# claussss/ubisoft-laforge-daft-exprt

Measured on AMD Instinct MI355X. Metric: mel frames/sec (fwd+bwd), higher is better.
Workload: dtype bf16; 1 GPU; C2: LJ-shaped training step, 48 utterances/GPU, L_max=120, T_max=896, 28180 valid frames/GPU/step; forward + loss (mel L1/L2, adversarial CE, post-mult, energy + pitch consistency) + backward + fused Adam step (global-norm clip, LR schedule) + one-launch weight re-pack, dropout on; parallelism=dp1, launch=1 captured HIP graph(s) per step (one per backward phase) + eager optimiser

## Files before the change

### include/daft_exprt_hip.h

```cpp
#ifndef DAFT_EXPRT_HIP_H
#define DAFT_EXPRT_HIP_H

#include <stdint.h>

#ifdef __cplusplus
extern "C" {
#endif

int dx_version(void);
const char* dx_last_error(void);
int dx_prof_enable(int kind, int capacity);
int dx_prof_collect(int kind, int* launches, double* total_ms);

int dx_int_durations(const float* dur, int B, int L, int sampling_rate, int filter_length, int hop_length, int centered,
                     long long* out, long long* totals, int* status);

int dx_pack_dims(int Cout, int Cin, int bf16, int* dims);
int dx_pack_weights(const float* W, void* fwd, void* bwd, int Cout, int Cin, int taps, int bf16, void* stream);
int dx_pack_weights_batched(const void* descs, int n, int bf16, void* stream);
int dx_pack_weights_host(const void* descs, int n, int bf16, void* stream);
int dx_conv_gemm(const void* X, int ldx, const void* Wp, const float* bias, void* Y, int ldy,
                 int B, int N, int Cin, int Cout, int taps, int bf16,
                 int relu, const float* post_scale, const float* post_shift,
                 const void* relu_aux, int ld_aux, int accumulate,
// ... 26 lines not shown
                     uint64_t seed_pre, float p_pre, const uint64_t* seed_offset, void* stream);
int dx_ff_block_bwd(const float* dY2, const float* z2, const float* mean2, const float* rstd2, const float* ln2_w, const float* ln2_b,
                    const float* film, int ld_film, void* DG2, float* dw2, float* db2, float* dfilm, int ld_dfilm, uint64_t seed2, float p2,
                    const void* Wa, const void* Wb, const void* aux, int ld_aux, void* H, int ldh, float* Y,
                    int B, int N, int F, const int* lens, int skip_halo,
                    const float* z1, const float* mean1, const float* rstd1, const float* ln1_w, const float* ln1_b, void* DG1, float* dw1, float* db1,
                    uint64_t seed1, float p1, const void* Wout_bwd, void* DATT, const uint64_t* seed_offset, const void* hmask,
                    const int* rows_exist, void* stream);
int dx_colsum(const void* X, int ldx, float* out, long rows, int C, int x_bf16, void* stream);

int dx_length_order(const int* lens, int* order, int B, void* stream);
int dx_attention_fwd(const void* qkv, int ld, const int* lens, void* ctx, int ldc, float* lse,
                     int B, int N, int H, int D, uint64_t seed, const uint64_t* seed_offset, float p_drop, int bf16, int qkv_bf16, int ctx_bf16,
                     const int* order, void* stream);
int dx_attention_proj_ln_fwd(const void* qkv, int ld, const int* lens, void* ctx, int ldc, float* lse, int B, int N, int H, int D,
                             uint64_t seed, const uint64_t* seed_offset, float p_drop,
                             const void* Wpack, const float* proj_bias, float* z, const float* res, const float* w, const float* bias,
                             const float* film, int ld_film, float* y, float* mean, float* rstd, uint64_t seed_pre, float p_pre,
                             void* y_bf16_copy, void* stream);
int dx_attention_bwd(const void* qkv, int ld, const void* ctx, const void* dctx, int ldc, const float* lse, float* delta,
                     const int* lens, void* dqkv, int ldg, int B, int N, int H, int D, uint64_t seed, const uint64_t* seed_offset, float p_drop, int bf16,
                     int qkv_bf16, int dqkv_bf16, int ctx_bf16, const int* order, void* stream);

int dx_ln_fwd(void* a, const void* res, const float* w, const float* bias, const float* film, int ld_film,
              const int* lens, int halo, void* y, float* mean, float* rstd, int B, int N, int C,
              uint64_t seed_pre, float p_pre, uint64_t seed_post, float p_post, const uint64_t* seed_offset, int io_bf16, void* y_bf16_copy,
              void* stream);
int dx_film_affine_fwd(const float* gammas, const float* betas, const float* pm, float* film, int B, int nb, int C, void* stream);
int dx_film_affine_bwd(const void* dfilm_ptrs, const float* gammas, const float* betas, const float* pm, float* dgammas, float* dbetas, float* dpm,
                       int B, int nb, int C, void* stream);
int dx_proj_ln_fwd(const void* X, int ldx, const void* Wpack, const float* proj_bias, float* z, const float* res, const float* w, const float* bias,
                   const float* film, int ld_film, const int* lens, int halo, float* y, float* mean, float* rstd, int B, int N,
                   uint64_t seed_pre, float p_pre, const uint64_t* seed_offset, void* y_bf16_copy, void* stream);
int dx_ln_bwd(const void* dy, const void* z, const float* mean, const float* rstd, const float* w, const float* bias,
              const float* film, int ld_film, const int* lens, int halo, void* dz, void* da, float* dw, float* dbias,
              float* dfilm, int ld_dfilm, int B, int N, int C, int relu_mask,
              uint64_t seed_pre, float p_pre, uint64_t seed_post, float p_post, const uint64_t* seed_offset, int io_bf16, void* dg_bf16_copy,
              void* stream);

int dx_add_pos(const float* x, const long* sym, const float* emb, const float* pe, const int* lens, float* out,
               int B, int N, int D, int pe_rows, void* stream);
int dx_mask_rows(const float* in, const int* lens, float* out, int B, int N, int C, void* stream);
int dx_embedding_bwd(const float* dout, const long* sym, const int* lens, float* demb, int B, int N, int D, void* stream);
int dx_accent_sum(const float* prenet, const float* energy, const float* pitch, const float* we, const float* be,
                  const float* wp, const float* bp, const float* pe, const int* lens, float* out,
                  int B, int N, int D, int pe_rows, void* stream);
int dx_scalar_conv_wgrad(const float* dout, int ldd, const float* rowscale, const float* s0, const float* s1, const int* lens,
                         float* dw0, float* db0, float* dw1, float* db1, int B, int N, int D, void* stream);
int dx_mean_pool(const float* x, const int* lens, float* out, int B, int N, int C, void* stream);
int dx_mean_pool_bwd(const float* dout, const int* lens, float* dx, int B, int N, int C, void* stream);
int dx_transpose(const float* in, float* out, int B, int R, int Cc, int accumulate, void* stream);
int dx_relu_bwd(const float* dy, const float* y, float* out, long n, void* stream);
int dx_channel_affine(const void* x, const float* scale, const float* shift, void* out, long rows, int C, int io_bf16, void* stream);
int dx_l2_normalize(const float* x, float* y, int rows, int C, void* stream);
int dx_cross_entropy(const float* logits, const long* target, float* loss, float* dlogits, int B, int S, void* stream);

int dx_duration_scan(const long* dur_int, float* mu, long* totals, int B, int L, void* stream);
int dx_upsample_prep(const float* enc, const float* dur, const float* energy, const float* pitch,
                     const float* wd, const float* bd, const float* we, const float* be, const float* wp, const float* bp,
                     const float* wr, const float* br, const int* lens, float* xs, float* z, float* sigma,
                     int B, int L, int D, void* stream);
int dx_upsample_fwd(const float* xs, const float* mu, const float* sigma, const int* lens, float* weights, float* xup,
                    int B, int L, int T, int D, void* stream);
int dx_upsample_bwd(const float* dxup, const float* xs, const float* mu, const float* sigma, const float* weights, const int* lens,
                    float* dxs, float* dsigma, int B, int L, int T, int D, void* stream);
int dx_upsample_sym_bwd(const float* dxs_in, const float* dsigma, const float* xs, const float* z, const float* dur, const int* lens,
// ... 62 lines not shown
```

### ubisoft_laforge_daft_exprt_amd/csrc/dx_f16_names.h

```cpp
#pragma once
#define dx_accent_sum dx_accent_sum_f16
#define dx_add_pos dx_add_pos_f16
#define dx_attention_bwd dx_attention_bwd_f16
#define dx_attention_fwd dx_attention_fwd_f16
#define dx_attention_proj_ln_fwd dx_attention_proj_ln_fwd_f16
#define dx_channel_affine dx_channel_affine_f16
#define dx_colsum dx_colsum_f16
#define dx_condition_prosody dx_condition_prosody_f16
#define dx_conv_gemm dx_conv_gemm_f16
#define dx_conv_wgrad dx_conv_wgrad_f16
#define dx_conv_wgrad_batched dx_conv_wgrad_batched_f16
#define dx_cross_entropy dx_cross_entropy_f16
#define dx_embedding_bwd dx_embedding_bwd_f16
#define dx_ff_block_bwd dx_ff_block_bwd_f16
#define dx_ff_pair dx_ff_pair_f16
#define dx_ff_pair_ln dx_ff_pair_ln_f16
#define dx_ff_pair_ln_qkv dx_ff_pair_ln_qkv_f16
#define dx_ff_pair_lnbwd dx_ff_pair_lnbwd_f16
#define dx_gather_speaker_rows dx_gather_speaker_rows_f16
#define dx_l2_normalize dx_l2_normalize_f16
#define dx_length_order dx_length_order_f16
#define dx_ln_bwd dx_ln_bwd_f16
#define dx_film_affine_bwd dx_film_affine_bwd_f16
#define dx_film_affine_fwd dx_film_affine_fwd_f16
#define dx_ln_fwd dx_ln_fwd_f16
#define dx_proj_ln_fwd dx_proj_ln_fwd_f16
#define dx_mask_rows dx_mask_rows_f16
#define dx_mean_pool dx_mean_pool_f16
#define dx_mean_pool_bwd dx_mean_pool_bwd_f16
#define dx_pack_dims dx_pack_dims_f16
#define dx_pitch_chain_bwd dx_pitch_chain_bwd_f16
#define dx_pitch_chain_fwd dx_pitch_chain_fwd_f16
#define dx_pack_weights dx_pack_weights_f16
#define dx_pack_weights_batched dx_pack_weights_batched_f16
#define dx_pack_weights_host dx_pack_weights_host_f16
#define dx_relu_bwd dx_relu_bwd_f16
#define dx_scalar_conv_wgrad dx_scalar_conv_wgrad_f16
#define dx_transpose dx_transpose_f16
#define dx_unpack_wgrad dx_unpack_wgrad_f16
```

### ubisoft_laforge_daft_exprt_amd/csrc/dx_gemm.hip

```cpp
#include "dx_common.h"
#include <algorithm>
#include <stdlib.h>
#include <type_traits>

namespace {

constexpr int TILE = 128;
constexpr int DK_MAX_B = 1024;

struct ConvGemmArgs {
  const float* X; int ldx;
  const void* Wp;
  const float* bias;
  float* Y; int ldy;
  int B, N, Cin, Cout, CinP, CoutP;
  int relu;
  const float* post_scale; const float* post_shift;
  const float* relu_aux; int ld_aux;
  int accumulate;
  const int* lens; int mask_rows;
  float out_scale;
  int skip_halo;
  int x_bf16, y_bf16, aux_bf16;
  const int* rows_exist;
// ... 1857 lines not shown
  long rr = r0;
  for (; rr + 3 < r1; rr += 4) {
    s0 += (float)X[(size_t)rr * ldx + c];
    s1 += (float)X[(size_t)(rr + 1) * ldx + c];
    s2 += (float)X[(size_t)(rr + 2) * ldx + c];
    s3 += (float)X[(size_t)(rr + 3) * ldx + c];
  }
  for (; rr < r1; ++rr) s0 += (float)X[(size_t)rr * ldx + c];
  const float t = (s0 + s1) + (s2 + s3);
  if (t != 0.f) atomicAdd(&out[c], t);
}

template <typename T, int TAPS, int TOK, bool XH>
void launch_conv_inst(const ConvGemmArgs& a, hipStream_t s) {
  const size_t smem = (size_t)(TAPS * TILE + TOK + TAPS - 1) * 128;
  static bool configured = false;
  if (!configured) {
    hipFuncSetAttribute(reinterpret_cast<const void*>(&conv_gemm_kernel<T, TAPS, TOK, XH>), hipFuncAttributeMaxDynamicSharedMemorySize, (int)smem);
    configured = true;
  }
  dim3 grid(a.B * dx_cdiv(a.N, TOK), a.CoutP / TILE);
  hipLaunchKernelGGL((conv_gemm_kernel<T, TAPS, TOK, XH>), grid, dim3(256), smem, s, a);
}

template <typename T, int TAPS>
int launch_conv(const ConvGemmArgs& a, hipStream_t s) {
  constexpr long small_below = (sizeof(T) == 4 || TAPS == 1) ? 1024 : 0;
  const bool small = (long)a.B * dx_cdiv(a.N, TILE) * (a.CoutP / TILE) < small_below;
  if constexpr (sizeof(T) == 2) {
    if (a.x_bf16) { if (small) launch_conv_inst<T, TAPS, 64, true>(a, s); else launch_conv_inst<T, TAPS, 128, true>(a, s); return DX_OK; }
  }
  if (small) launch_conv_inst<T, TAPS, 64, false>(a, s); else launch_conv_inst<T, TAPS, 128, false>(a, s);
  return DX_OK;
}

}

extern "C" {

int dx_pack_dims(int Cout, int Cin, int bf16, int* dims) {
  const int bk = bf16 ? 64 : 32;
  dims[0] = dx_roundup(Cout, TILE);
  dims[1] = dx_roundup(Cin, bk);
  dims[2] = dx_roundup(Cin, TILE);
  dims[3] = dx_roundup(Cout, bk);
  return DX_OK;
}

int dx_pack_weights(const float* W, void* fwd, void* bwd, int Cout, int Cin, int taps, int bf16, void* stream) {
  DX_REQUIRE(W && fwd, "dx_pack_weights: null pointer");
  DX_REQUIRE(Cout > 0 && Cin > 0 && (taps == 1 || taps == 3), "dx_pack_weights: bad dims Cout=%d Cin=%d taps=%d", Cout, Cin, taps);
  int d[4];
  dx_pack_dims(Cout, Cin, bf16, d);
  const size_t n = (size_t)taps * d[0] * d[1] + (bwd ? (size_t)taps * d[2] * d[3] : 0);
  const int blocks = (int)std::min<size_t>((n + 255) / 256, 4096);
  hipStream_t s = (hipStream_t)stream;
  if (bf16)
    hipLaunchKernelGGL(pack_weights_kernel<dx_h16>, dim3(blocks), dim3(256), 0, s, W, (dx_h16*)fwd, (dx_h16*)bwd, Cout, Cin, taps, d[0], d[1], d[2], d[3]);
  else
    hipLaunchKernelGGL(pack_weights_kernel<float>, dim3(blocks), dim3(256), 0, s, W, (float*)fwd, (float*)bwd, Cout, Cin, taps, d[0], d[1], d[2], d[3]);
  DX_LAUNCH_CHECK("dx_pack_weights");
  return DX_OK;
}

int dx_pack_weights_batched(const void* descs, int n, int bf16, void* stream) {
  DX_REQUIRE(descs && n > 0, "dx_pack_weights_batched: bad arguments");
// ... 47 lines not shown
  DX_REQUIRE(!aux_bf16 || ((Cout % 4) == 0 && (ld_aux % 4) == 0), "dx_conv_gemm: bf16 relu_aux needs Cout, ld_aux multiples of 4");
  DX_REQUIRE(skip_halo < 0 || lens, "dx_conv_gemm: skip_halo needs lens");
  DX_REQUIRE(B > 0 && N > 0 && Cin > 0 && Cout > 0, "dx_conv_gemm: bad dims B=%d N=%d Cin=%d Cout=%d", B, N, Cin, Cout);
  DX_REQUIRE(taps == 1 || taps == 3, "dx_conv_gemm: taps must be 1 or 3 (got %d)", taps);
  DX_REQUIRE((Cin % 4) == 0 && (ldx % 4) == 0 && ldx >= Cin, "dx_conv_gemm: Cin (%d) and ldx (%d) must be multiples of 4, ldx >= Cin", Cin, ldx);
  DX_REQUIRE(ldy >= Cout && ((Cout % 4) != 0 || (ldy % 4) == 0), "dx_conv_gemm: bad ldy %d for Cout %d", ldy, Cout);
  DX_REQUIRE(((uintptr_t)X % 16) == 0 && ((uintptr_t)Wp % 16) == 0 && ((uintptr_t)Y % 16) == 0, "dx_conv_gemm: pointers must be 16-byte aligned");
  DX_REQUIRE(!relu_aux || ld_aux >= Cout, "dx_conv_gemm: bad ld_aux");
  DX_REQUIRE((post_scale == nullptr) == (post_shift == nullptr), "dx_conv_gemm: post_scale/post_shift must come together");
  DX_REQUIRE(!mask_rows || lens, "dx_conv_gemm: mask_rows needs lens");
  int d[4];
  dx_pack_dims(Cout, Cin, bf16 == 1, d);
  ConvGemmArgs a{X, ldx, Wp, bias, Y, ldy, B, N, Cin, Cout, d[1], d[0], relu, post_scale, post_shift,
                 relu_aux, ld_aux, accumulate, lens, mask_rows, out_scale, skip_halo, x_bf16, y_bf16, aux_bf16, rows_exist};
  hipStream_t s = (hipStream_t)stream;
  dx_prof_begin(DX_PROF_CONV_GEMM, s);
  constexpr int ws_min_tiles = 64;
  constexpr int dk_min_cin = 256;
  if (bf16 == 2) {
    if constexpr (kSplitBuild) { if (taps == 3) launch_conv<dx_split3, 3>(a, s); else launch_conv<dx_split3, 1>(a, s); }
  } else if (bf16 && d[1] >= dk_min_cin && (Cin % 64) == 0 && (long)B * N * ldx < (1L << 31)) {
    if (x_bf16) { if (taps == 3) launch_conv_dk<3, true>(a, s); else launch_conv_dk<1, true>(a, s); }
    else { if (taps == 3) launch_conv_dk<3, false>(a, s); else launch_conv_dk<1, false>(a, s); }
  } else if (bf16 && d[1] == 128 && (long)B * dx_cdiv(N, 128) >= ws_min_tiles) {
    if (x_bf16) { if (taps == 3) launch_conv_ws<3, true>(a, s); else launch_conv_ws<1, true>(a, s); }
    else { if (taps == 3) launch_conv_ws<3, false>(a, s); else launch_conv_ws<1, false>(a, s); }
  } else if (bf16) { if (taps == 3) launch_conv<dx_h16, 3>(a, s); else launch_conv<dx_h16, 1>(a, s); }
  else      { if (taps == 3) launch_conv<float, 3>(a, s);  else launch_conv<float, 1>(a, s); }
  dx_prof_end(DX_PROF_CONV_GEMM, s);
  DX_LAUNCH_CHECK("dx_conv_gemm");
  return DX_OK;
}

int dx_conv_wgrad(const void* dY, int ldy, const void* X, int ldx, float* G,
                  int B, int N, int Cin, int Cout, int taps, const int* lens, int skip_halo,
                  int bf16, int dy_bf16, int x_bf16, float* dbias, const int* rows_exist, void* stream) {
  DX_REQUIRE(dY && X && G, "dx_conv_wgrad: null pointer");
  DX_REQUIRE(bf16 == 0 || bf16 == 1 || (bf16 == 2 && kSplitBuild), "dx_conv_wgrad: bad operand mode %d", bf16);
  DX_REQUIRE(bf16 == 1 || !(dy_bf16 || x_bf16), "dx_conv_wgrad: bf16 storage needs bf16 operand mode");
  const bool bf16_ok = (Cin % 8) == 0 && (ldx % 8) == 0 && (Cout % 8) == 0 && (ldy % 8) == 0;
  DX_REQUIRE(bf16_ok || !(dy_bf16 || x_bf16), "dx_conv_wgrad: bf16-stored operands need Cin/Cout/ld multiples of 8 (Cin=%d Cout=%d)", Cin, Cout);
  if (bf16 == 1 && bf16_ok) {
    DX_REQUIRE(B > 0 && N > 0 && Cin > 0 && Cout > 0 && (taps == 1 || taps == 3), "dx_conv_wgrad: bad dims");
    DX_REQUIRE(((uintptr_t)X % 16) == 0 && ((uintptr_t)dY % 16) == 0, "dx_conv_wgrad: pointers must be 16-byte aligned");
    DX_REQUIRE(skip_halo < 0 || lens, "dx_conv_wgrad: skip_halo needs lens");
    const bool wide = (Cin % 128) == 0 && dx_cdiv(Cout, TILE) * dx_cdiv(Cin, 64) >= 64;
    const int tiles = dx_cdiv(Cout, TILE) * dx_cdiv(Cin, wide ? 128 : 64);
    const int total_chunks = B * dx_cdiv(N, wb_bk(taps, dy_bf16 != 0, x_bf16 != 0));
    constexpr int target_blocks = 256;
    constexpr int target_wide = 256;
    constexpr int target_k1 = 192;
    const int ksplit = std::max(1, std::min(total_chunks, dx_cdiv(wide ? target_wide : (taps == 1 ? target_k1 : target_blocks), tiles)));
    WgradBatchArgs a{};
    a.job[0] = WgradJobDev{dY, X, G, dbias, lens, ldy, ldx, B, N, Cin, Cout, skip_halo, 0, rows_exist};
    a.ksplit = ksplit;
    hipStream_t s = (hipStream_t)stream;
    dim3 grid(tiles, 1, ksplit);
    dx_prof_begin(DX_PROF_WGRAD_GEMM, s);
#define DX_WG_LAUNCH(TAPS_, CIW_)                                                                                        \
    if (dy_bf16 && x_bf16) hipLaunchKernelGGL((wgrad_bf16_kernel<TAPS_, true, true, CIW_>), grid, dim3(CIW_ * 128), 0, s, a);   \
    else if (dy_bf16) hipLaunchKernelGGL((wgrad_bf16_kernel<TAPS_, true, false, CIW_>), grid, dim3(CIW_ * 128), 0, s, a);       \
    else if (x_bf16) hipLaunchKernelGGL((wgrad_bf16_kernel<TAPS_, false, true, CIW_>), grid, dim3(CIW_ * 128), 0, s, a);        \
    else hipLaunchKernelGGL((wgrad_bf16_kernel<TAPS_, false, false, CIW_>), grid, dim3(CIW_ * 128), 0, s, a);
    if (wide) { if (taps == 3) { DX_WG_LAUNCH(3, 4) } else { DX_WG_LAUNCH(1, 4) } }
    else { if (taps == 3) { DX_WG_LAUNCH(3, 2) } else { DX_WG_LAUNCH(1, 2) } }
#undef DX_WG_LAUNCH
// ... 94 lines not shown
```

### ubisoft_laforge_daft_exprt_amd/functional.py

```python
from __future__ import annotations

import threading

import torch

from . import ops

_seed_state = threading.local()


def manual_seed(seed: int) -> None:
    _seed_state.base = (int(seed) * 0x9E3779B97F4A7C15 + 0x1234567) & 0xFFFFFFFFFFFFFFFF
    _seed_state.counter = 0


def next_seed() -> int:
    if not hasattr(_seed_state, 'base'):
        manual_seed(torch.initial_seed())
    _seed_state.counter += 1
    return (_seed_state.base + _seed_state.counter * 0xD1B54A32D192ED03) & 0xFFFFFFFFFFFFFFFF


def _sink(param, enabled):
    if not enabled or param is None:
# ... 197 lines not shown
            dz1, da1, dln1_w, dln1_b = r1[:4]
            dproj = r1[5] if sh else (da1 if da1 is not None else dz1)
        dc1_w, dc1_b = ops.conv_wgrad(dh, y1, packs['c1'], L, 1, arena=arena, w_sink=g('c1_w'), b_sink=g('c1_b'), prec=prec, defer=True, rows_exist=E)
        dout_w, dout_b = ops.conv_wgrad(dproj, att, packs['out'], L, 0, arena=arena, w_sink=g('out_w'), b_sink=g('out_b'), prec=prec, defer=True)
        if datt is None:
            datt = ops.conv_gemm(dproj, packs['out'], None, transpose=True, lens=L, halo=0, prec=prec, out_dtype=att.dtype)
        dqkv = ops.attention_bwd(qkv, att, datt, lse, L, ctx.heads, s_attn, p_attn, out_dtype=qkv.dtype, prec=prec, seed_offset=so)
        din_w, din_b = ops.conv_wgrad(dqkv, x, packs['in'], L, 0, arena=arena, w_sink=g('in_w'), b_sink=g('in_b'), prec=prec, defer=True)
        dx = ops.conv_gemm(dqkv, packs['in'], None, transpose=True, out=dz1, accumulate=True, lens=L, halo=0, prec=prec)
        return (dx, dfilm, None, None, None, None,
                din_w, din_b, dout_w, dout_b, dln1_w, dln1_b, dc1_w, dc1_b, dc2_w, dc2_b, dln2_w, dln2_b, None, None)


def cut(rt, level, t):
    sp = None if rt is None else rt.backward_split
    if sp is None or level > rt.cut_levels or not t.requires_grad:
        return t
    leaf = t.detach().requires_grad_(True)
    sp.append((level, t, leaf))
    return leaf


class AccentFront0Fn(torch.autograd.Function):
    @staticmethod
    def forward(ctx, mel, lens, packs, p_drop, training, c0_w, c0_b, l0_w, l0_b):
        p = p_drop if training else 0.0
        seed = next_seed() if training else 0
        x0 = ops.transpose(mel.contiguous())
        L = lens.i32
        rt = packs['p0'].rt
        prec = rt.precision
        hd = ops.hidden_dtype(prec)
        so = rt.seed_offset
        h0 = ops.conv_gemm(x0, packs['p0'], c0_b, relu=True, lens=L, halo=2, out_dtype=hd, prec=prec, rows_exist=lens.exist)
        y0, m0, r0 = ops.ln_fwd(h0, None, l0_w, l0_b, None, L, seed_post=seed, p_post=p, halo=2, seed_offset=so, prec=prec)
        ctx.save_for_backward(x0, h0, m0, r0, l0_w, l0_b)
        ctx.lens, ctx.packs, ctx.p, ctx.seed = lens, packs, p, seed
        ctx.prec, ctx.sink, ctx.seed_offset = prec, rt.sink, so
        return y0

    @staticmethod
    def backward(ctx, dy0):
        x0, h0, m0, r0, l0_w, l0_b = ctx.saved_tensors
        lens, packs, p = ctx.lens, ctx.packs, ctx.p
        arena = packs['p0'].rt.arena
        L = lens.i32
        sk = {k: _sink(v, ctx.sink) for k, v in packs.get('params', {}).items()}
        g = sk.get
        dz0, _, dl0_w, dl0_b, _ = ops.ln_bwd(dy0.contiguous(), h0, m0, r0, l0_w, l0_b, None, L, relu_mask=True, seed_post=ctx.seed, p_post=p,
                                              seed_offset=ctx.seed_offset, prec=ctx.prec, w_sink=g('l0_w'), b_sink=g('l0_b'), halo=2, arena=arena)
        dc0_w, dc0_b = ops.conv_wgrad(dz0, x0, packs['p0'], L, 2, w_sink=g('c0_w'), b_sink=g('c0_b'), prec=ctx.prec, arena=arena, rows_exist=lens.exist)
        return None, None, None, None, None, dc0_w, dc0_b, dl0_w, dl0_b


class AccentFront12Fn(torch.autograd.Function):
    @staticmethod
    def forward(ctx, y0, energy, pitch, lens, packs, pe, p_drop, training,
                c1_w, c1_b, l1_w, l1_b, c2_w, c2_b, l2_w, l2_b, we, be, wp, bp):
        p = p_drop if training else 0.0
        seeds = [next_seed() if training else 0 for _ in range(2)]
        L = lens.i32
        rt = packs['p1'].rt
        prec = rt.precision
        hd = ops.hidden_dtype(prec)
        so = rt.seed_offset
        h1 = ops.conv_gemm(y0, packs['p1'], c1_b, relu=True, lens=L, halo=1, out_dtype=hd, prec=prec, rows_exist=lens.exist)
        y1, m1, r1 = ops.ln_fwd(h1, None, l1_w, l1_b, None, L, seed_post=seeds[0], p_post=p, halo=1, seed_offset=so, prec=prec)
        h2 = ops.conv_gemm(y1, packs['p2'], c2_b, relu=True, lens=L, halo=0, prec=prec, rows_exist=lens.exist)
# ... 164 lines not shown
```

### ubisoft_laforge_daft_exprt_amd/ops.py

```python
from __future__ import annotations

import ctypes

import torch

from . import _lib
from ._lib import lib

PRECISIONS = ('f32', 'bf16', 'fp16', 'bf16x3')


class Runtime:

    def __init__(self, precision='f32'):
        self.precision = _check_precision(precision)
        self.pack_epoch = 0
        self.sink = False
        self.launch_log = None
        self.arena = None
        self.arena_hint = 1 << 20
        self.seed_offset = None
        self.defer_wgrad = False
        self.wgrad_queue = {}
        self.backward_split = None
# ... 464 lines not shown
    return ctx, lse


def attention_bwd(qkv, ctx, dctx, lse, lens, heads, seed, p_drop, out_dtype=torch.float32, prec=None, seed_offset=None, order=None):
    B, N, D3 = qkv.shape
    D = D3 // 3
    if dctx.dtype != ctx.dtype:
        raise TypeError(f'ctx ({ctx.dtype}) and dctx ({dctx.dtype}) must be stored alike')
    dqkv = torch.empty(B, N, D3, dtype=out_dtype, device=qkv.device)
    delta = torch.empty(B, heads, N, dtype=torch.float32, device=qkv.device)
    prec = prec or DEFAULT.precision
    _fn('dx_attention_bwd', prec)(_p(qkv), _rows(qkv), _p(ctx), _p(dctx), _rows(dctx), _p(lse), _p(delta), _p(lens), _p(dqkv), _rows(dqkv),
                           B, N, heads, D, seed, _p(seed_offset), float(p_drop), _mode(prec), _is_bf16(qkv), _is_bf16(dqkv), _is_bf16(ctx),
                           _p(order), _stream())
    return dqkv


def gemm_shadow(prec=None):
    return bool(_half(prec or DEFAULT.precision))


def ln_fwd(a, res, w, b, film, lens, *, seed_pre=0, p_pre=0.0, seed_post=0, p_post=0.0, halo=0, shadow=False, seed_offset=None, prec=None):
    B, N, C = a.shape
    y = torch.empty_like(a)
    prec = prec or DEFAULT.precision
    y_h = torch.empty(B, N, C, dtype=_H16[prec], device=a.device) if shadow else None
    mean = torch.empty(B, N, dtype=torch.float32, device=a.device)
    rstd = torch.empty(B, N, dtype=torch.float32, device=a.device)
    _fn('dx_ln_fwd', prec)(_p(a), _p(res), _p(w), _p(b), _p(film), 0 if film is None else film.stride(0), _p(lens), int(halo), _p(y), _p(mean), _p(rstd),
                    B, N, C, seed_pre, float(p_pre), seed_post, float(p_post), _p(seed_offset), _is_bf16(a), _p(y_h), _stream())
    return (y, mean, rstd, y_h) if shadow else (y, mean, rstd)


def attn_proj_ln_applies(qkv, heads, pack: PackedWeight, prec) -> bool:
    return (prec in _H16 and qkv.dtype == _H16[prec] and qkv.dim() == 3 and qkv.shape[2] == 384 and heads == 2
            and pack.taps == 1 and pack.cin == 128 and pack.cout == 128)


def attn_proj_ln_fwd(qkv, lens, heads, seed, p_drop, pack: PackedWeight, proj_bias, res, w, b, film, *, seed_pre=0, p_pre=0.0, shadow=False,
                     seed_offset=None, prec=None):
    B, N, D3 = qkv.shape
    D = D3 // 3
    prec = prec or pack.rt.precision
    _check_h16(prec, qkv)
    h16 = _H16[prec]
    ctx = torch.empty(B, N, D, dtype=h16, device=qkv.device)
    lse = torch.empty(B, heads, N, dtype=torch.float32, device=qkv.device)
    z = torch.empty(B, N, D, dtype=torch.float32, device=qkv.device)
    y = torch.empty_like(z)
    y_h = torch.empty(B, N, D, dtype=h16, device=qkv.device) if shadow else None
    mean = torch.empty(B, N, dtype=torch.float32, device=qkv.device)
    rstd = torch.empty(B, N, dtype=torch.float32, device=qkv.device)
    img = pack.image(prec)
    _log(pack, ('gemm', B * N, N, pack.cin, pack.cout, 1))
    _fn('dx_attention_proj_ln_fwd', prec)(_p(qkv), _rows(qkv), _p(lens), _p(ctx), D, _p(lse), B, N, heads, D, seed, _p(seed_offset), float(p_drop),
                                          _p(img.fwd), _p(proj_bias), _p(z), _p(res), _p(w), _p(b), _p(film), 0 if film is None else film.stride(0),
                                          _p(y), _p(mean), _p(rstd), seed_pre, float(p_pre), _p(y_h), _stream())
    return (ctx, lse, z, y, mean, rstd, y_h) if shadow else (ctx, lse, z, y, mean, rstd)


def proj_ln_fwd(x, pack: PackedWeight, proj_bias, res, w, b, film, lens, *, seed_pre=0, p_pre=0.0, halo=0, shadow=False, seed_offset=None, prec=None):
    B, N, C = x.shape
    prec = prec or pack.rt.precision
    _check_h16(prec, x)
    img = pack.image(prec)
    z = torch.empty(B, N, C, dtype=torch.float32, device=x.device)
# ... 254 lines not shown
```

### ubisoft_laforge_daft_exprt_amd/profiling.py

```python
from __future__ import annotations

from collections import OrderedDict

PEAK_TFLOPS = {'f32': 157.3, 'bf16': 2500.0, 'bf16x3': 2500.0 / 3}
PEAK_HBM_GBS = 8000.0


class Geometry:

    def __init__(self, axes):
        self.by_n = {}
        for lens in axes:
            lens = [int(v) for v in lens]
            self.by_n[(len(lens), max(lens))] = (sum(lens), sum(v * v for v in lens))

    def rows(self, B, N, lens_ptr=True):
        if not lens_ptr:
            return B * N
        return self.by_n.get((B, N), (B * N, B * N * N))[0]

    def pairs(self, B, N):
        return self.by_n.get((B, N), (B * N, B * N * N))[1]


# ... 58 lines not shown
    if name == 'dx_conv_wgrad_batched':
        from . import ops
        jobs = ops.WGRAD_BATCH_LOG.get(a['jobs'], (None, []))[1]
        flops = byt = 0
        for (_dy, _x, _g, _db, lens, _ldy, _ldx, B, N, Cin, Cout, *_rest) in jobs:
            rows = geom.rows(B, N, lens is not None)
            flops += 2.0 * a['taps'] * Cin * Cout * rows
            byt += rows * (Cout * (2 if a['dy_bf16'] else 4) + Cin * (2 if a['x_bf16'] else 4)) + a['taps'] * Cin * Cout * 4
        return f"wgrad_bf16_kernel<{a['taps']},wide>", 'mfma', (flops or None), (byt or None)
    if name in ('dx_attention_fwd', 'dx_attention_bwd'):
        rows, pairs = geom.rows(a['B'], a['N']), geom.pairs(a['B'], a['N'])
        D, H = a['D'], a['H']
        qb = 2 if a['qkv_bf16'] else 4
        sfx = ' <bf16x3>' if a['bf16'] == 2 else ''
        if name == 'dx_attention_fwd':
            return 'attn_fwd' + sfx, 'mfma', 4.0 * pairs * D, rows * (3 * D * qb + D * 4 + H * 4)
        gb = 2 if a['dqkv_bf16'] else 4
        return 'attn_bwd (dq + dkv)' + sfx, 'mfma', 14.0 * pairs * D, rows * (2 * 3 * D * qb + 2 * D * 4 + 3 * D * gb + 2 * H * 4)
    if name in ('dx_pitch_chain_fwd', 'dx_pitch_chain_bwd'):
        rows = geom.rows(a['B'], a['T'], True)
        flops = 2.0 * 3 * (a['M'] * 256 + 2 * 256 * 256 + 256) * rows
        byt = rows * (a['M'] * 4 + 4 + 96 + (a['M'] * 8 if name.endswith('bwd') else 0))
        return ('pitch_chain<fwd>' if name.endswith('fwd') else 'pitch_chain<bwd>'), 'mfma', flops, byt
    if name == 'dx_attention_proj_ln_fwd':
        rows, pairs = geom.rows(a['B'], a['N']), geom.pairs(a['B'], a['N'])
        D, H = a['D'], a['H']
        byt = rows * (3 * D * 2 + D * 2 + H * 4) + rows * (128 * (4 + 4 + (4 if has('res') else 0) + (2 if has('y_bf16_copy') else 0)) + 8) + 128 * 128 * 2
        return 'attn_fwd+proj_ln', 'mfma', 4.0 * pairs * D + 2.0 * rows * 128 * 128, byt
    if name == 'dx_ln_fwd':
        rows = geom.rows(a['B'], a['N'], has('lens'))
        C, ab = a['C'], (2 if a['io_bf16'] else 4)
        byt = rows * (C * (2 * ab + 4 + (4 if has('res') else 0) + (2 if has('y_bf16_copy') else 0)) + 8)
        return f'ln_fwd_kernel<{C}>', 'hbm', None, byt
    if name == 'dx_proj_ln_fwd':
        rows = geom.rows(a['B'], a['N'], has('lens'))
        byt = rows * (128 * (2 + 4 + 4 + (4 if has('res') else 0) + (2 if has('y_bf16_copy') else 0)) + 8) + 128 * 128 * 2
        return 'proj_ln_fwd', 'hbm', None, byt
    if name == 'dx_ln_bwd':
        rows = geom.rows(a['B'], a['N'], has('lens'))
        C, zb = a['C'], (2 if a['io_bf16'] else 4)
        byt = rows * (C * (3 * zb + (4 if has('da') else 0) + (2 if has('dg_bf16_copy') else 0)) + 8)
        return f'ln_bwd_kernel<{C}>', 'hbm', None, byt
    if name == 'dx_upsample_fwd':
        B, L, T, D = a['B'], a['L'], a['T'], a['D']
        return 'upsample_fwd', 'hbm', None, B * L * D * 4 + 3 * B * L * 4 + B * T * D * 4 + B * L * T * 4
    if name == 'dx_upsample_bwd':
        B, L, T, D = a['B'], a['L'], a['T'], a['D']
        return 'upsample_bwd (dsigma + dxs)', 'hbm', None, B * T * D * 4 + B * L * T * 4 + 2 * B * L * D * 4 + 3 * B * L * 4
    if name in ('dx_upsample_prep', 'dx_upsample_sym_bwd'):
        return name[3:], 'hbm', None, 2 * a['B'] * a['L'] * a['D'] * 4 + 6 * a['B'] * a['L'] * 4
    if name == 'dx_adam_step':
        return 'adam_kernel', 'hbm', None, a['n'] * 28
    if name == 'dx_sumsq':
        return 'sumsq_kernel', 'hbm', None, a['n'] * 4
    if name == 'dx_mel_stats':
        return 'mel_stats', 'hbm', None, 2 * a['B'] * a['M'] * a['T'] * 4
    if name == 'dx_mel_grad':
        return 'mel_grad', 'hbm', None, 3 * a['B'] * a['M'] * a['T'] * 4
    if name == 'dx_add_pos':
        rows = geom.rows(a['B'], a['N'])
        return 'add_pos', 'hbm', None, rows * a['D'] * 4 * (2 if has('x') else 1)
    if name == 'dx_accent_sum':
        return 'accent_sum', 'hbm', None, geom.rows(a['B'], a['N']) * (2 * a['D'] * 4 + 8)
    if name == 'dx_scalar_conv_wgrad':
        return 'scalar_conv_wgrad', 'hbm', None, geom.rows(a['B'], a['N']) * (a['D'] * 4 if a['ldd'] else 0) + geom.rows(a['B'], a['N']) * 8
    if name == 'dx_transpose':
# ... 73 lines not shown
```

Before: 4.782 million valid mel frames/s.

## Fuse first prenet conv+ReLU with LayerNorm and dropout into one kernel

Adds a dedicated kernel for the first prenet layer that runs the 3-tap conv GEMM (fp32 input, Cin up to 128 to 1024 channels) with bias+ReLU, stages the result in LDS, then does LayerNorm and post-dropout in the same block. The goal is to drop one launch and the HBM round trip of the 1024-wide hidden activation between conv_gemm and ln_fwd. It still writes H for backward and skips tiles past the padded length. The risk is lower occupancy from the large LDS footprint and a less tuned GEMM than the generic path.

```diff
diff --git a/include/daft_exprt_hip.h b/include/daft_exprt_hip.h
--- a/include/daft_exprt_hip.h
+++ b/include/daft_exprt_hip.h
@@ -82,6 +82,9 @@
 int dx_proj_ln_fwd(const void* X, int ldx, const void* Wpack, const float* proj_bias, float* z, const float* res, const float* w, const float* bias,
                    const float* film, int ld_film, const int* lens, int halo, float* y, float* mean, float* rstd, int B, int N,
                    uint64_t seed_pre, float p_pre, const uint64_t* seed_offset, void* y_bf16_copy, void* stream);
+int dx_prenet_front0_fwd(const float* X, int ldx, const void* Wpack, const float* bias, const float* ln_w, const float* ln_b,
+                         const int* lens, const int* rows_exist, int halo, void* H, void* Y, float* mean, float* rstd,
+                         int B, int N, int Cin, int Cout, uint64_t seed_post, float p_post, const uint64_t* seed_offset, void* stream);
 int dx_ln_bwd(const void* dy, const void* z, const float* mean, const float* rstd, const float* w, const float* bias,
               const float* film, int ld_film, const int* lens, int halo, void* dz, void* da, float* dw, float* dbias,
               float* dfilm, int ld_dfilm, int B, int N, int C, int relu_mask,
diff --git a/ubisoft_laforge_daft_exprt_amd/csrc/dx_f16_names.h b/ubisoft_laforge_daft_exprt_amd/csrc/dx_f16_names.h
--- a/ubisoft_laforge_daft_exprt_amd/csrc/dx_f16_names.h
+++ b/ubisoft_laforge_daft_exprt_amd/csrc/dx_f16_names.h
@@ -25,6 +25,7 @@
 #define dx_film_affine_fwd dx_film_affine_fwd_f16
 #define dx_ln_fwd dx_ln_fwd_f16
 #define dx_proj_ln_fwd dx_proj_ln_fwd_f16
+#define dx_prenet_front0_fwd dx_prenet_front0_fwd_f16
 #define dx_mask_rows dx_mask_rows_f16
 #define dx_mean_pool dx_mean_pool_f16
 #define dx_mean_pool_bwd dx_mean_pool_bwd_f16
diff --git a/ubisoft_laforge_daft_exprt_amd/csrc/dx_gemm.hip b/ubisoft_laforge_daft_exprt_amd/csrc/dx_gemm.hip
--- a/ubisoft_laforge_daft_exprt_amd/csrc/dx_gemm.hip
+++ b/ubisoft_laforge_daft_exprt_amd/csrc/dx_gemm.hip
@@ -1913,6 +1913,172 @@
   }
   if (small) launch_conv_inst<T, TAPS, 64, false>(a, s); else launch_conv_inst<T, TAPS, 128, false>(a, s);
   return DX_OK;
+}
+
+#include "dx_rowvec.h"
+constexpr float F0_LN_EPS = 1e-5f;
+constexpr int F0_TOK = 32;
+constexpr int F0_C = 1024;
+constexpr int F0_HLD = F0_C * 2 + 16;
+
+struct Front0Args {
+  const float* X; int ldx;
+  const dx_h16* Wp;
+  const float* bias;
+  const float* ln_w; const float* ln_b;
+  const int* lens; const int* rows_exist;
+  int halo;
+  dx_h16* H; dx_h16* Y;
+  float* mean; float* rstd;
+  int B, N, Cin;
+  uint64_t seed_post; uint32_t thresh_post; float inv_keep_post;
+  const uint64_t* seed_offset;
+};
+
+template <int NKB>
+__global__ __launch_bounds__(512, 4) void prenet_front0_kernel(const Front0Args a) {
+  constexpr int TAPS = 3, PAD = 1, TOK = F0_TOK, C = F0_C;
+  constexpr int XROWS = TOK + TAPS - 1;
+  constexpr int XBUF = XROWS * 128;
+  constexpr int XU = 32;
+  constexpr int X_IT = (XROWS * XU + 511) / 512;
+  constexpr int NJ = TOK / 16;
+  constexpr int KBP = 4;
+  constexpr int E = RowVec<C>::E;
+  extern __shared__ __attribute__((aligned(16))) unsigned char smem[];
+  unsigned char* Xs = smem;
+  unsigned char* Hs = smem + 2 * XBUF;
+
+  const int tid = threadIdx.x, lane = tid & 63;
+  const int wave = __builtin_amdgcn_readfirstlane(tid >> 6);
+  const int r = lane & 15, g = lane >> 4;
+  const int tiles_n = (a.N + TOK - 1) / TOK;
+  const int b = blockIdx.x / tiles_n;
+  const int n0 = (blockIdx.x - b * tiles_n) * TOK;
+  const int len_h = a.lens[b] + a.halo;
+
+  if ((n0 & ~127) >= len_h) {
+    for (int rr = wave; rr < TOK && n0 + rr < a.N; rr += 8) {
+      const size_t row = (size_t)b * a.N + n0 + rr;
+#pragma unroll
+      for (int k = 0; k < RowVec<C>::K; ++k) {
+        *reinterpret_cast<uint2*>(a.H + row * C + (k * 64 + lane) * 4) = make_uint2(0u, 0u);
+        *reinterpret_cast<uint2*>(a.Y + row * C + (k * 64 + lane) * 4) = make_uint2(0u, 0u);
+      }
+      if (lane == 0) { a.mean[row] = 0.f; a.rstd[row] = 0.f; }
+    }
+    return;
+  }
+
+  const int NL = a.rows_exist ? min(a.rows_exist[b], a.N) : a.N;
+#pragma unroll
+  for (int it = 0; it < X_IT; ++it) {
+    const int u = tid + it * 512;
+    const int row = u >> 5, q = u & 31;
+    const int n = n0 + row - PAD, ci = q * 4;
+    if (u < XROWS * XU && q < NKB * 8) {
+      f32x4 v = f32x4{0.f, 0.f, 0.f, 0.f};
+      if (n >= 0 && n < NL && ci < a.Cin) v = *reinterpret_cast<const f32x4*>(a.X + ((size_t)b * a.N + n) * a.ldx + ci);
+      *reinterpret_cast<uint2*>(Xs + (q >> 4) * XBUF + lds_off(row, (q & 15) >> 1) + ((q & 1) << 3)) = pack_bf16x4v(v);
+    }
+  }
+  __syncthreads();
+
+  const dx_h16* const wwave = a.Wp + (size_t)(wave * 8) * KBP * 512;
+  const int wlane = lane * 8;
+  constexpr int wtap = (C >> 4) * KBP * 512;
+  f32x4 acc[8][NJ];
+#pragma unroll
+  for (int i = 0; i < 8; ++i)
+#pragma unroll
+    for (int j = 0; j < NJ; ++j) acc[i][j] = f32x4{0.f, 0.f, 0.f, 0.f};
+  constexpr int NSTEP = TAPS * NKB;
+  float4 wf[2][4], xf[NJ];
+#define F0_STEP_TAP(T_) ((T_) < 2 * TAPS ? (T_) / 2 : ((T_) - 2 * TAPS) / (NKB - 2))
+#define F0_STEP_KB(T_) ((T_) < 2 * TAPS ? (T_) % 2 : 2 + ((T_) - 2 * TAPS) % (NKB - 2))
+#define F0_LOAD_W(HS_)                                                                                                           \
+  {                                                                                                                              \
+    const int t_ = (HS_) >> 1, h_ = (HS_) & 1;                                                                                   \
+    _Pragma("unroll") for (int i = 0; i < 4; ++i) {                                                                              \
+      int off_ = F0_STEP_TAP(t_) * wtap + ((h_ * 4 + i) * KBP + F0_STEP_KB(t_)) * 512;                                           \
+      asm volatile("" : "+s"(off_));           \
+      wf[(HS_) & 1][i] = *reinterpret_cast<const float4*>(wwave + off_ + wlane);                                                 \
+    }                                                                                                                            \
+  }
+  F0_LOAD_W(0)
+#pragma unroll
+  for (int hs = 0; hs < 2 * NSTEP; ++hs) {
+    if (hs + 1 < 2 * NSTEP) F0_LOAD_W(hs + 1)
+    const int t = hs >> 1, half = hs & 1;
+    const int tap = F0_STEP_TAP(t), kb = F0_STEP_KB(t);
+    if (half == 0) {
+#pragma unroll
+      for (int j = 0; j < NJ; ++j) xf[j] = *reinterpret_cast<const float4*>(Xs + (kb >> 1) * XBUF + lds_off(j * 16 + r + tap, (kb & 1) * 4 + g));
+    }
+#pragma unroll
+    for (int i = 0; i < 4; ++i)
+#pragma unroll
+      for (int j = 0; j < NJ; ++j) Mma<dx_h16>::run(wf[hs & 1][i], xf[j], acc[half * 4 + i][j]);
+    __builtin_amdgcn_sched_barrier(0);
+  }
+#undef F0_LOAD_W
+#undef F0_STEP_TAP
+#undef F0_STEP_KB
+
+#pragma unroll
+  for (int i = 0; i < 8; ++i) {
+    const int cl = wave * 128 + i * 16 + g * 4;
+    float bv[4] = {0.f, 0.f, 0.f, 0.f};
+    if (a.bias) { const float4 tb = *reinterpret_cast<const float4*>(a.bias + cl); bv[0] = tb.x; bv[1] = tb.y; bv[2] = tb.z; bv[3] = tb.w; }
+#pragma unroll
+    for (int j = 0; j < NJ; ++j) {
+      const int tok = j * 16 + r;
+      float v[4];
+#pragma unroll
+      for (int e = 0; e < 4; ++e) v[e] = fmaxf(acc[i][j][e] + bv[e], 0.f) + 0.f;
+      if (n0 + tok >= NL) { v[0] = v[1] = v[2] = v[3] = 0.f; }
+      *reinterpret_cast<uint2*>(Hs + tok * F0_HLD + cl * 2) = pack_bf16x4(make_float4(v[0], v[1], v[2], v[3]));
+    }
+  }
+  __syncthreads();
+
+  const int l = __lane_id();
+  uint64_t seed_post = a.seed_post;
+  if (a.seed_offset) seed_post += *a.seed_offset;
+  float wv[E], lb[E];
+#pragma unroll
+  for (int e = 0; e < E; ++e) { wv[e] = a.ln_w[row_col<C>(l, e)]; lb[e] = a.ln_b[row_col<C>(l, e)]; }
+  for (int rr = wave; rr < TOK && n0 + rr < a.N; rr += 8) {
+    const int n = n0 + rr;
+    const size_t row = (size_t)b * a.N + n;
+    const bool valid = n < len_h;
+    float z[E];
+    row_load<C>(reinterpret_cast<const dx_h16*>(Hs + rr * F0_HLD), l, z);
+    row_store<C>(a.H + row * C, l, z);
+    if (!valid) {
+#pragma unroll
+      for (int e = 0; e < E; ++e) z[e] = 0.f;
+    }
+    float s = 0.f;
+#pragma unroll
+    for (int e = 0; e < E; ++e) s += z[e];
+    const float mu = row_sum<C>(s) * (1.0f / C);
+    float q = (z[1] - mu) * (z[1] - mu);
+    q = __builtin_fmaf(z[0] - mu, z[0] - mu, q);
+#pragma unroll
+    for (int e = 2; e < E; ++e) { const float d = z[e] - mu; q = __builtin_fmaf(d, d, q); }
+    const float rs = 1.0f / sqrtf(row_sum<C>(q) * (1.0f / C) + F0_LN_EPS);
+    if (l == 0) { a.mean[row] = valid ? mu : 0.f; a.rstd[row] = valid ? rs : 0.f; }
+    float y[E], fpost[E];
+    if (a.thresh_post) row_dropout<C>(seed_post, (uint64_t)row, l, a.thresh_post, a.inv_keep_post, fpost);
+#pragma unroll
+    for (int e = 0; e < E; ++e) {
+      float t = __builtin_fmaf((z[e] - mu) * rs, wv[e], lb[e]);
+      if (a.thresh_post) t *= fpost[e];
+      y[e] = valid ? t : 0.f;
+    }
+    row_store<C>(a.Y + row * C, l, y);
+  }
 }
 
 }
@@ -2026,6 +2192,37 @@
   return DX_OK;
 }
 
+int dx_prenet_front0_fwd(const float* X, int ldx, const void* Wp, const float* bias, const float* ln_w, const float* ln_b,
+                         const int* lens, const int* rows_exist, int halo, void* H, void* Y, float* mean, float* rstd,
+                         int B, int N, int Cin, int Cout, uint64_t seed_post, float p_post, const uint64_t* seed_offset, void* stream) {
+  DX_REQUIRE(X && Wp && ln_w && ln_b && lens && H && Y && mean && rstd, "dx_prenet_front0_fwd: null pointer");
+  DX_REQUIRE(B > 0 && N > 0 && halo >= 0, "dx_prenet_front0_fwd: bad dims");
+  DX_REQUIRE(Cout == F0_C && Cin > 64 && Cin <= 128 && (Cin % 4) == 0, "dx_prenet_front0_fwd: built for 64 < Cin <= 128 (multiple of 4) -> 1024 (got %d -> %d)", Cin, Cout);
+  DX_REQUIRE((ldx % 4) == 0 && ldx >= Cin, "dx_prenet_front0_fwd: ldx (%d) must be a multiple of 4, >= Cin", ldx);
+  DX_REQUIRE(((uintptr_t)X % 16) == 0 && ((uintptr_t)Wp % 16) == 0 && ((uintptr_t)H % 16) == 0 && ((uintptr_t)Y % 16) == 0 &&
+             (!bias || ((uintptr_t)bias % 16) == 0), "dx_prenet_front0_fwd: pointers must be 16-byte aligned");
+  DX_REQUIRE(p_post >= 0.f && p_post < 1.f, "dx_prenet_front0_fwd: dropout p out of range");
+  DX_REQUIRE((long)B * dx_cdiv(N, F0_TOK) < (1L << 31), "dx_prenet_front0_fwd: too many token tiles");
+  Front0Args k{X, ldx, (const dx_h16*)Wp, bias, ln_w, ln_b, lens, rows_exist, halo, (dx_h16*)H, (dx_h16*)Y, mean, rstd, B, N, Cin,
+               seed_post, (uint32_t)lrintf(p_post * 65536.f), 1.f / (1.f - p_post), seed_offset};
+  hipStream_t s = (hipStream_t)stream;
+  const size_t smem = (size_t)2 * (F0_TOK + 2) * 128 + (size_t)F0_TOK * F0_HLD;
+  const dim3 grid(B * dx_cdiv(N, F0_TOK));
+  dx_prof_begin(DX_PROF_CONV_GEMM, s);
+  if (Cin <= 96) {
+    static bool configured = false;
+    if (!configured) { hipFuncSetAttribute(reinterpret_cast<const void*>(&prenet_front0_kernel<3>), hipFuncAttributeMaxDynamicSharedMemorySize, (int)smem); configured = true; }
+    hipLaunchKernelGGL(prenet_front0_kernel<3>, grid, dim3(512), smem, s, k);
+  } else {
+    static bool configured = false;
+    if (!configured) { hipFuncSetAttribute(reinterpret_cast<const void*>(&prenet_front0_kernel<4>), hipFuncAttributeMaxDynamicSharedMemorySize, (int)smem); configured = true; }
+    hipLaunchKernelGGL(prenet_front0_kernel<4>, grid, dim3(512), smem, s, k);
+  }
+  dx_prof_end(DX_PROF_CONV_GEMM, s);
+  DX_LAUNCH_CHECK("dx_prenet_front0_fwd");
+  return DX_OK;
+}
+
 int dx_conv_wgrad(const void* dY, int ldy, const void* X, int ldx, float* G,
                   int B, int N, int Cin, int Cout, int taps, const int* lens, int skip_halo,
                   int bf16, int dy_bf16, int x_bf16, float* dbias, const int* rows_exist, void* stream) {
diff --git a/ubisoft_laforge_daft_exprt_amd/functional.py b/ubisoft_laforge_daft_exprt_amd/functional.py
--- a/ubisoft_laforge_daft_exprt_amd/functional.py
+++ b/ubisoft_laforge_daft_exprt_amd/functional.py
@@ -253,8 +253,12 @@
         prec = rt.precision
         hd = ops.hidden_dtype(prec)
         so = rt.seed_offset
-        h0 = ops.conv_gemm(x0, packs['p0'], c0_b, relu=True, lens=L, halo=2, out_dtype=hd, prec=prec, rows_exist=lens.exist)
-        y0, m0, r0 = ops.ln_fwd(h0, None, l0_w, l0_b, None, L, seed_post=seed, p_post=p, halo=2, seed_offset=so, prec=prec)
+        if ops.prenet_front0_applies(x0, packs['p0'], prec):
+            h0, y0, m0, r0 = ops.prenet_front0_fwd(x0, packs['p0'], c0_b, l0_w, l0_b, L, halo=2, seed_post=seed, p_post=p, seed_offset=so, prec=prec,
+                                                   rows_exist=lens.exist)
+        else:
+            h0 = ops.conv_gemm(x0, packs['p0'], c0_b, relu=True, lens=L, halo=2, out_dtype=hd, prec=prec, rows_exist=lens.exist)
+            y0, m0, r0 = ops.ln_fwd(h0, None, l0_w, l0_b, None, L, seed_post=seed, p_post=p, halo=2, seed_offset=so, prec=prec)
         ctx.save_for_backward(x0, h0, m0, r0, l0_w, l0_b)
         ctx.lens, ctx.packs, ctx.p, ctx.seed = lens, packs, p, seed
         ctx.prec, ctx.sink, ctx.seed_offset = prec, rt.sink, so
diff --git a/ubisoft_laforge_daft_exprt_amd/ops.py b/ubisoft_laforge_daft_exprt_amd/ops.py
--- a/ubisoft_laforge_daft_exprt_amd/ops.py
+++ b/ubisoft_laforge_daft_exprt_amd/ops.py
@@ -520,6 +520,31 @@
     return (y, mean, rstd, y_h) if shadow else (y, mean, rstd)
 
 
+def prenet_front0_applies(x, pack: PackedWeight, prec) -> bool:
+    return (prec in _H16 and x.dtype == torch.float32 and x.dim() == 3 and pack.taps == 3 and pack.cout == 1024
+            and 64 < pack.cin <= 128 and pack.cin % 4 == 0)
+
+
+def prenet_front0_fwd(x, pack: PackedWeight, bias, w, b, lens, *, halo=0, seed_post=0, p_post=0.0, seed_offset=None, prec=None, rows_exist=None):
+    _chk(x, 'x')
+    prec = prec or pack.rt.precision
+    if not prenet_front0_applies(x, pack, prec):
+        raise TypeError('prenet_front0_fwd serves a 16-bit operand mode, fp32 input and a (1024, 64 < Cin <= 128, 3) weight')
+    img = pack.image(prec)
+    B, N, cin = x.shape
+    if cin != pack.cin:
+        raise ValueError(f'expected {pack.cin} input channels, got {cin}')
+    dt = _H16[prec]
+    h = torch.empty(B, N, pack.cout, dtype=dt, device=x.device)
+    y = torch.empty_like(h)
+    mean = torch.empty(B, N, dtype=torch.float32, device=x.device)
+    rstd = torch.empty(B, N, dtype=torch.float32, device=x.device)
+    _log(pack, ('conv', B * N, N, cin, pack.cout, pack.taps))
+    _fn('dx_prenet_front0_fwd', prec)(_p(x), _rows(x), _p(img.fwd), _p(bias), _p(w), _p(b), _p(lens), _p(rows_exist), int(halo), _p(h), _p(y),
+                                      _p(mean), _p(rstd), B, N, cin, pack.cout, seed_post, float(p_post), _p(seed_offset), _stream())
+    return h, y, mean, rstd
+
+
 def attn_proj_ln_applies(qkv, heads, pack: PackedWeight, prec) -> bool:
     return (prec in _H16 and qkv.dtype == _H16[prec] and qkv.dim() == 3 and qkv.shape[2] == 384 and heads == 2
             and pack.taps == 1 and pack.cin == 128 and pack.cout == 128)
diff --git a/ubisoft_laforge_daft_exprt_amd/profiling.py b/ubisoft_laforge_daft_exprt_amd/profiling.py
--- a/ubisoft_laforge_daft_exprt_amd/profiling.py
+++ b/ubisoft_laforge_daft_exprt_amd/profiling.py
@@ -114,6 +114,9 @@
         C, ab = a['C'], (2 if a['io_bf16'] else 4)
         byt = rows * (C * (2 * ab + 4 + (4 if has('res') else 0) + (2 if has('y_bf16_copy') else 0)) + 8)
         return f'ln_fwd_kernel<{C}>', 'hbm', None, byt
+    if name == 'dx_prenet_front0_fwd':
+        rows = geom.rows(a['B'], a['N'], True)
+        return 'prenet_front0_kernel', 'hbm', 2.0 * 3 * a['Cin'] * a['Cout'] * rows, rows * (a['Cin'] * 4 + 2 * a['Cout'] * 2 + 8) + 3 * a['Cin'] * a['Cout'] * 2
     if name == 'dx_proj_ln_fwd':
         rows = geom.rows(a['B'], a['N'], has('lens'))
         byt = rows * (128 * (2 + 4 + 4 + (4 if has('res') else 0) + (2 if has('y_bf16_copy') else 0)) + 8) + 128 * 128 * 2
```

Result: no change. 4.822 million valid mel frames/s, median of 6 (+0.8%).
